# mrvollger/rustybam

Measured on AMD Instinct MI355X. Metric: CIGAR-ops/s, liftover over 100 kb sliding windows (whole pass, inputs resident in HBM), higher is better.
Workload: dtype u32

## Files before the change

### rustybam_amd/csrc/capi.hip

```cpp
#include <hip/hip_runtime.h>
#include <sys/mman.h>

#include <algorithm>
#include <cstdarg>
#include <cstdio>
#include <cstdlib>
#include <cstring>
#include <ctime>
#include <numeric>
#include <string>
#include <thread>
#include <vector>
#include <chrono>
#include <map>
#include <mutex>

#include "../../include/rustybam_amd.h"
#include "rb_lift.h"
#include "rb_trim.h"
#include "rb_launch.h"

#ifndef RB_SCAN_ROWS_MEAN_MAX
#define RB_SCAN_ROWS_MEAN_MAX 1536
#endif
#ifndef RB_SHORT_MAX_DEFAULT
#define RB_SHORT_MAX_DEFAULT 2048
#endif

#define RB_MAX_ARENA 256

#define RB_TIMING_RING 256
__global__ __launch_bounds__(256) void rb_k_fill_bytes(uint8_t *dst, uint32_t v4, size_t n) {
    const uintptr_t a = (uintptr_t)dst;
    const size_t head = n < 16 ? n : (size_t)((16 - (a & 15)) & 15);
    const size_t body = (n - head) / 16;
    const size_t tail0 = head + body * 16;
    const size_t i = (size_t)blockIdx.x * blockDim.x + threadIdx.x, stride = (size_t)gridDim.x * blockDim.x;
    for (size_t k = i; k < body; k += stride) *reinterpret_cast<uint4 *>(dst + head + k * 16) = make_uint4(v4, v4, v4, v4);
    if (i < head) dst[i] = (uint8_t)v4;
    if (i < n - tail0) dst[tail0 + i] = (uint8_t)v4;
}
extern "C" hipError_t rb_fill_async(void *dst, int value, size_t bytes, hipStream_t stream) {
    if (!bytes) return hipSuccess;
    const uint32_t b = (uint32_t)value & 255u, v4 = b | (b << 8) | (b << 16) | (b << 24);
    const size_t groups = bytes / 16 + 1;
    const unsigned blocks = (unsigned)std::min<size_t>((groups + 255) / 256, 65536);
    hipLaunchKernelGGL(rb_k_fill_bytes, dim3(blocks ? blocks : 1), dim3(256), 0, stream, (uint8_t *)dst, v4, bytes);
    return hipGetLastError();
}

struct rb_ctx {
    int device = -1;
    hipStream_t stream = nullptr;
    bool own_stream = false;
    std::string err;
    bool timing = false;
    std::vector<hipEvent_t> ev_a, ev_b;
    uint64_t timed_calls = 0;
    void *trim_scratch = nullptr;
    uint32_t trim_scratch_blocks = 0;
    void *trim_pend = nullptr;
    uint64_t trim_pend_cap = 0;
    void *scan_list = nullptr;
    uint64_t scan_list_cap = 0;
    uint64_t scan_rows_n = 0;
    void *pin[2] = {nullptr, nullptr};
    hipEvent_t pin_ev[2] = {nullptr, nullptr};
    bool pin_busy[2] = {false, false};
    unsigned pin_next = 0;
    uint64_t alloc_fallbacks = 0;
// ... 639 lines not shown
    if (!rc) rc = upload_vec(ctx, g_orig, &pl->w_orig);
    if (!rc) rc = upload_vec(ctx, o_st, &pl->wo_st);
    if (!rc) rc = upload_vec(ctx, o_en, &pl->wo_en);
    if (!rc) rc = upload_vec(ctx, cw_off, &pl->cw_off);
    if (!rc) rc = upload_vec(ctx, mono, &pl->cw_mono);
    if (!rc && pl->n_tiles) rc = upload_vec(ctx, tiles, &pl->tiles);
    if (!rc && hipStreamSynchronize(ctx->stream) != hipSuccess) rc = fail(ctx, RB_E_HIP, "plan upload: %s", hipGetErrorString(hipGetLastError()));
    if (rc) {
        rb_plan_destroy(pl);
        return rc;
    }
    *out = pl;
    return RB_OK;
}
extern "C" void rb_plan_destroy(rb_plan *pl) {
    if (!pl) return;
    void *ptrs[] = {pl->sched, pl->slot_of, pl->ident, pl->canon_pos, pl->w_st, pl->w_en, pl->w_orig, pl->wo_st, pl->wo_en, pl->cw_off, pl->cw_mono, pl->tiles};
    for (void *q : ptrs)
        if (q) (void)rb_dev_free(pl->ctx, q);
    delete pl;
}

struct ws_layout {
    size_t hit_off, win_lo, block_sums, arena, pend_count, pend_list, jobs, gen_list, x_st, x_en, bp_tmp, bp_off, bp_cur, brk_rows, copy_count, copy_list, decl_count, decl_list, gen_cp, diag_stamps, fb_count, fb_list, starts_bad, total;
};
static bool rb_no_gen_cp() {
    static const bool v = getenv("RB_DEBUG_NO_GEN_CP") != nullptr;
    return v;
}
static ws_layout ws_of(uint64_t n_rec, uint64_t rows_cap, uint64_t n_ops) {
    ws_layout w;
    size_t o = 0;
    auto take = [&](size_t bytes) {
        size_t at = o;
        o += (bytes + 255) & ~(size_t)255;
        return at;
    };
    w.hit_off = take((n_rec + 2) * 8);
    w.win_lo = take((n_rec + 2) * 4);
    w.block_sums = take(rb_scan_block_sums_count(n_rec) * 8);
    w.arena = take((size_t)RB_MAX_ARENA * RB_ARENA_STRIDE * 8);
    w.pend_count = take(256);
    w.pend_list = take((n_rec + 1) * 4);
    w.jobs = take((n_rec + 1) * sizeof(rb_job));
    w.gen_list = take((rows_cap + 1) * 4);
    w.x_st = take((rows_cap + 1) * 8);
    w.x_en = take((rows_cap + 1) * 8);
    w.bp_tmp = take((rows_cap + 1) * 8);
    w.bp_off = take((n_rec + 1) * 8);
    w.bp_cur = take((size_t)RB_MAX_ARENA * 128);
    w.brk_rows = take((rows_cap + 1) * sizeof(rb_hit_row));
    w.copy_count = take(256);
    w.copy_list = take((rows_cap + 1) * 16);
    w.decl_count = take(256);
    w.decl_list = take((n_rec + 1) * 4);
    w.gen_cp = take(rb_no_gen_cp() ? 256 : (size_t)(n_ops / RB_GCP + n_rec + 2) * sizeof(uint4));
    w.diag_stamps = take((n_rec + 1) * 4);
    w.fb_count = take(256);
    w.fb_list = take((n_rec + 1) * 4);
    w.starts_bad = take(256);
    w.total = o;
    return w;
}
extern "C" size_t rb_plan_workspace_bytes(const rb_plan *plan, uint64_t rows_cap) {
    if (!plan) return 0;
    return ws_of(plan->n_rec, rows_cap, plan->n_ops).total;
}
extern "C" size_t rb_plan_diag_stamps_offset(const rb_plan *plan, uint64_t rows_cap) {
    if (!plan) return 0;
    return ws_of(plan->n_rec, rows_cap, plan->n_ops).diag_stamps;
}

static uint64_t slot_stride_of(uint64_t n_ops, uint64_t n_rec) { return ((n_ops + 31) & ~(uint64_t)31) + 32 * n_rec + 64; }
extern "C" uint64_t rb_plan_out_capacity(const rb_plan *plan, int for_break) {
    if (!plan) return 0;
    const uint64_t slots = for_break ? std::min<uint32_t>(2u, RB_MS) : std::min<uint32_t>(plan->depth, RB_MS);
    return slots * slot_stride_of(plan->n_ops, plan->n_rec) + plan->n_ops / 16 + 32 * plan->n_rec + (1u << 20);
}

static uint32_t pick_arenas(uint64_t n_rec) {
    uint64_t a = n_rec / 256;
// ... 62 lines not shown
    p.op_starts = (policy & RB_LIFT_OP_STARTS) ? 1 : 0;
    if (p.op_starts && p.fused) return fail(ctx, RB_E_INVALID, "RB_LIFT_OP_STARTS takes finished norm_rows: not together with RB_LIFT_FUSED_SCAN");
    if (p.op_starts && (policy & RB_LIFT_DESCRIPTORS)) return fail(ctx, RB_E_INVALID, "RB_LIFT_OP_STARTS with RB_LIFT_DESCRIPTORS: a descriptor indexes the record's ORIGINAL cigar, which a batch cut in place no longer is");
    if (p.op_starts && b->n_ops > plan->n_ops) return fail(ctx, RB_E_INVALID, "RB_LIFT_OP_STARTS: batch->n_ops exceeds the plan's op count (gather the batch first)");
    if (p.op_starts && b->n_rec) {
        unsigned long long *bad = (unsigned long long *)(ws + w.starts_bad), first_bad = 0;
        HIPCHK(ctx, rb_fill_async(bad, 0xFF, 8, ctx->stream));
        HIPCHK(ctx, rb_launch_starts_check(b->op_off, norm, b->n_rec, b->n_ops, bad, ctx->stream));
        HIPCHK(ctx, hipMemcpyAsync(&first_bad, bad, 8, hipMemcpyDeviceToHost, ctx->stream));
        HIPCHK(ctx, hipStreamSynchronize(ctx->stream));
        if (first_bad != ~0ull)
            return fail(ctx, RB_E_INVALID, "RB_LIFT_OP_STARTS: record %llu lies outside the batch's %llu ops (a pass moved it: gather the batch first)",
                        first_bad, (unsigned long long)b->n_ops);
    }
    p.norm_w = const_cast<rb_norm_row *>(norm);
    p.pend_list = (uint32_t *)(ws + w.pend_list);
    p.pend_count = (unsigned long long *)(ws + w.pend_count);
    const bool use_tiles = plan->n_tiles != 0 && ((policy >> 8) & 0xFFF) == 0;
    p.tile_first = use_tiles ? plan->tiles : nullptr;
    p.n_tiles = use_tiles ? plan->n_tiles : 0;
    p.fb_list = (uint32_t *)(ws + w.fb_list);
    p.fb_count = (unsigned long long *)(ws + w.fb_count);
    const uint32_t stream_end = use_tiles ? plan->stream_end : (uint32_t)b->n_rec;
    rb_scan_params sp;
    memset(&sp, 0, sizeof sp);
    if (p.fused) {
        sp.n_rec = b->n_rec;
        sp.ops = b->ops;
        sp.op_off = b->op_off;
        sp.t_st = b->t_st, sp.t_en = b->t_en, sp.q_st = b->q_st, sp.q_en = b->q_en;
        sp.strand = b->strand;
        sp.norm_rows = p.norm_w;
        HIPCHK(ctx, rb_fill_async(p.pend_count, 0, 8, ctx->stream));
        HIPCHK(ctx, rb_launch_peek_norm(&sp, ctx->stream));
    }
    p.counters = counters;
    p.policy = policy & 1;
    p.early_exit = (policy & RB_LIFT_EARLY_EXIT) ? 1 : 0;
    p.debug_skip = (policy >> 8) & 0xFFF;
    uint64_t *block_sums = (uint64_t *)(ws + w.block_sums);
    HIPCHK(ctx, rb_fill_async(counters, 0, sizeof(rb_counters), ctx->stream));
    HIPCHK(ctx, rb_fill_async(p.copy_count, 0, 8, ctx->stream));
    HIPCHK(ctx, rb_fill_async(p.arena_cur, 0, (size_t)RB_MAX_ARENA * RB_ARENA_STRIDE * 8, ctx->stream));
    if (b->n_rec == 0) return RB_OK;
    const bool one_walk = is_break && (policy & RB_BREAK_ONE_WALK) && !p.desc_mode;
    if (one_walk) {
        p.brk_mode = 1, p.brk_max = max_size;
        p.rows_final = rows;
        p.rows = (rb_hit_row *)(ws + w.brk_rows);
        p.brk_off = (uint64_t *)(ws + w.bp_off);
        p.brk_cursor = (unsigned long long *)(ws + w.bp_cur);
        p.brk_n_arena = pick_arenas(b->n_rec);
        p.brk_arena_cap = rows_cap / p.brk_n_arena;
        p.brk_decl_list = (uint32_t *)(ws + w.decl_list);
        p.brk_decl_count = (unsigned long long *)(ws + w.decl_count);
        HIPCHK(ctx, rb_fill_async(p.brk_decl_count, 0, 8, ctx->stream));
        HIPCHK(ctx, rb_fill_async(p.brk_cursor, 0, (size_t)RB_MAX_ARENA * 128, ctx->stream));
        HIPCHK(ctx, rb_fill_async(p.hit_off, 0, (size_t)(b->n_rec + 2) * 8, ctx->stream));
        HIPCHK(ctx, rb_fill_async(p.brk_off, 0xFF, (size_t)(b->n_rec + 1) * 8, ctx->stream));
        HIPCHK(ctx, rb_launch_make_jobs(&p, ctx->stream));
        const size_t slot1 = (size_t)(ctx->timed_calls % RB_TIMING_RING);
        if (ctx->timing) HIPCHK(ctx, hipEventRecord(ctx->ev_a[slot1], ctx->stream));
        p.wave0 = 0;
        p.wave_end = stream_end;
        HIPCHK(ctx, rb_launch_liftover_stream(&p, ctx->stream));
        if (use_tiles) {
            HIPCHK(ctx, rb_fill_async(p.fb_count, 0, 8, ctx->stream));
            HIPCHK(ctx, rb_launch_liftover_tiles(&p, ctx->stream));
            HIPCHK(ctx, rb_launch_liftover_stream_list(&p, ctx->stream));
        }
        if (p.fused) {
            sp.list = p.pend_list;
            sp.n_list = (const uint64_t *)p.pend_count;
            HIPCHK(ctx, rb_launch_scan_records(&sp, ctx->stream));
        }
        if (ctx->timing) {
            HIPCHK(ctx, hipEventRecord(ctx->ev_b[slot1], ctx->stream));
            ctx->timed_calls++;
        }
        rb_break_params bp;
        memset(&bp, 0, sizeof bp);
        bp.n_rec = b->n_rec, bp.ops = b->ops, bp.op_off = b->op_off, bp.norm = norm, bp.sched = plan->sched, bp.hit_off = p.hit_off;
        bp.x_st = (uint64_t *)(ws + w.x_st), bp.x_en = (uint64_t *)(ws + w.x_en);
        bp.rows_cap = rows_cap, bp.max_size = max_size;
        bp.list = p.brk_decl_list, bp.n_list = p.brk_decl_count;
        bp.fill = 0;
        HIPCHK(ctx, rb_launch_break_list_declined(&p, ctx->stream));
        HIPCHK(ctx, rb_launch_break_pieces(&bp, ctx->stream));
        HIPCHK(ctx, rb_launch_count_and_scan(&p, block_sums, false, ctx->stream));
        bp.fill = 1;
        HIPCHK(ctx, rb_launch_break_pieces(&bp, ctx->stream));
        HIPCHK(ctx, rb_launch_break_gather(&p, ctx->stream));
        rb_lift_params pg = p;
        pg.rows = rows, pg.x_st = bp.x_st, pg.x_en = bp.x_en;
        HIPCHK(ctx, rb_launch_break_declined(&pg, ctx->stream));
        return RB_OK;
    }
    if (is_break) {
        rb_break_params bp;
        memset(&bp, 0, sizeof bp);
        bp.n_rec = b->n_rec;
        bp.ops = b->ops;
        bp.op_off = b->op_off;
        bp.norm = norm;
        bp.sched = plan->sched;
        bp.hit_off = p.hit_off;
        bp.x_st = (uint64_t *)(ws + w.x_st);
        bp.x_en = (uint64_t *)(ws + w.x_en);
        bp.rows_cap = rows_cap;
        bp.max_size = max_size;
        bp.tmp = (uint2 *)(ws + w.bp_tmp);
        bp.tmp_off = (uint64_t *)(ws + w.bp_off);
        bp.tmp_cursor = (unsigned long long *)(ws + w.bp_cur);
        bp.n_arena = pick_arenas(b->n_rec);
        bp.arena_cap = rows_cap / bp.n_arena;
        HIPCHK(ctx, rb_fill_async(bp.tmp_cursor, 0, (size_t)RB_MAX_ARENA * 128, ctx->stream));
        bp.fill = 2, bp.redo_only = 0;
        HIPCHK(ctx, rb_launch_break_pieces(&bp, ctx->stream));
        HIPCHK(ctx, rb_launch_count_and_scan(&p, block_sums, false, ctx->stream));
        HIPCHK(ctx, rb_launch_break_place(&bp, ctx->stream));
        bp.fill = 1, bp.redo_only = 1;
        HIPCHK(ctx, rb_launch_break_pieces(&bp, ctx->stream));
        p.x_st = bp.x_st;
        p.x_en = bp.x_en;
    } else {
        HIPCHK(ctx, rb_launch_count_and_scan(&p, block_sums, true, ctx->stream));
    }
    HIPCHK(ctx, rb_launch_make_jobs(&p, ctx->stream));
    const size_t slot = (size_t)(ctx->timed_calls % RB_TIMING_RING);
    if (ctx->timing) HIPCHK(ctx, hipEventRecord(ctx->ev_a[slot], ctx->stream));
    p.wave0 = 0;
    p.wave_end = stream_end;
    HIPCHK(ctx, rb_launch_liftover_stream(&p, ctx->stream));
    if (use_tiles) {
        HIPCHK(ctx, rb_fill_async(p.fb_count, 0, 8, ctx->stream));
        HIPCHK(ctx, rb_launch_liftover_tiles(&p, ctx->stream));
        HIPCHK(ctx, rb_launch_liftover_stream_list(&p, ctx->stream));
    }
    if (p.fused) {
        sp.list = p.pend_list;
        sp.n_list = (const uint64_t *)p.pend_count;
        HIPCHK(ctx, rb_launch_scan_records(&sp, ctx->stream));
    }
    if (ctx->timing) {
        HIPCHK(ctx, hipEventRecord(ctx->ev_b[slot], ctx->stream));
        ctx->timed_calls++;
    }
    HIPCHK(ctx, rb_launch_liftover_tail(&p, ctx->stream));
    return RB_OK;
}

extern "C" int rb_dev_liftover(rb_ctx *ctx, const rb_plan *plan, const rb_batch_view *batch, const rb_norm_row *norm_rows,
                               int bsearch_policy, void *workspace, rb_hit_row *rows, uint64_t rows_cap, uint32_t *out_ops,
                               uint64_t out_cap, rb_counters *counters) {
    return lift_common(ctx, plan, batch, norm_rows, bsearch_policy, workspace, rows, rows_cap, out_ops, out_cap, counters, false, 0);
}
extern "C" int rb_dev_break(rb_ctx *ctx, const rb_plan *plan, const rb_batch_view *batch, const rb_norm_row *norm_rows,
                            uint32_t max_size, int bsearch_policy, void *workspace, rb_hit_row *rows, uint64_t rows_cap,
// ... 1117 lines not shown
```

### rustybam_amd/csrc/k_liftover.hip

```cpp
#include "rb_lift.h"
#include "rb_launch.h"
#include <type_traits>
#include <algorithm>

__global__ __launch_bounds__(256) void rb_k_count_hits(rb_lift_params p) {
    const uint64_t r = (uint64_t)blockIdx.x * blockDim.x + threadIdx.x;
    if (r >= p.n_rec) return;
    uint64_t cnt = 0;
    const rb_norm_row *nr = &p.norm[r];
    const uint32_t c = p.contig[r];
    if (nr->status == RB_ST_OK && c < p.n_contig) {
        const uint64_t ws = p.cw_off[c], we = p.cw_off[c + 1];
        const uint64_t t_st = nr->t_st, t_en = nr->t_en;
        if (p.cw_mono[c]) {
            const uint64_t lo = rb_lower_en_gt(p.w_en, ws, we, t_st);
            const uint64_t hi = rb_lower_st_ge(p.w_st, ws, we, t_en);
            cnt = hi > lo ? hi - lo : 0;
            p.win_lo[r] = (uint32_t)lo;
        } else {
            for (uint64_t i = ws; i < we; i++) cnt += (t_en > p.w_st[i] && t_st < p.w_en[i]) ? 1 : 0;
        }
    }
    p.hit_off[p.canon_pos[r]] = cnt;
}

#define RB_SCAN_PER_BLOCK 2048
__global__ __launch_bounds__(256) void rb_k_scan_partial(const uint64_t *v, uint64_t n, uint64_t *block_sums) {
    __shared__ uint64_t sh[4];
    const uint64_t base = (uint64_t)blockIdx.x * RB_SCAN_PER_BLOCK;
    uint64_t s = 0;
    for (int k = 0; k < RB_SCAN_PER_BLOCK / 256; k++) {
        uint64_t i = base + (uint64_t)k * 256 + threadIdx.x;
        if (i < n) s += v[i];
    }
    s = rb_wave_sum_u64(s);
    if ((threadIdx.x & 63) == 0) sh[threadIdx.x >> 6] = s;
    __syncthreads();
    if (threadIdx.x == 0) block_sums[blockIdx.x] = sh[0] + sh[1] + sh[2] + sh[3];
}
__global__ __launch_bounds__(256) void rb_k_scan_top(uint64_t *block_sums, uint64_t n_blocks) {
    __shared__ uint64_t sh[256];
    __shared__ uint64_t carry;
    if (threadIdx.x == 0) carry = 0;
    __syncthreads();
    for (uint64_t b = 0; b < n_blocks; b += 256) {
        uint64_t i = b + threadIdx.x;
        uint64_t x = i < n_blocks ? block_sums[i] : 0;
// ... 56 lines not shown
    j.n = nr->n_ops;
    j.rec0 = p.op_off[r] + nr->first_op;
    j.t_st = nr->t_st, j.t_en = nr->t_en, j.q_st = nr->q_st, j.q_en = nr->q_en;
    const uint64_t k = p.canon_pos[r];
    const bool brk = p.brk_mode != 0;
    const uint64_t h0 = brk ? 0ull : p.hit_off[k], nh = brk ? 1ull : p.hit_off[k + 1] - h0;
    const bool explicit_w = brk || p.x_st != nullptr;
    const uint32_t cg = p.contig[r];
    const bool mono = explicit_w || (cg < p.n_contig && p.cw_mono[cg] != 0);
    uint32_t f = 0;
    const bool provisional = (nr->flags & RB_F_PROVISIONAL) != 0;
    if (nr->status == RB_ST_OK && (nh != 0 || provisional)) {
        if (h0 + nh > p.rows_cap) f |= RB_JOB_ROWS_OVERFLOW;
        else f |= RB_JOB_VALID;
    }
    if ((nr->flags & RB_F_REGULAR) || (provisional && !(nr->flags & RB_F_ENDS_NOT_MATCH))) f |= RB_JOB_REGULAR;
    if (p.strand[r] == (uint8_t)'-') f |= RB_JOB_MINUS;
    if (mono) f |= RB_JOB_MONO;
    j.flags = f;
    j.h0 = (uint32_t)h0;
    j.nh = (uint32_t)nh;
    j.lo = (explicit_w || !mono || !(f & RB_JOB_VALID) || nh == 0) ? 0u : p.win_lo[r];
    p.jobs[w] = j;
}

#define RB_RING_BASE 88
#define RB_RING_TOP_N 103
#define RB_SPILL_ROOM 4
#define RB_WPE 4, 5
#include "rb_stream.h"
#define RB_STREAM_KERNEL(NAME, BRK, DIAG, ROOM)                                                                                   \
    __global__ __launch_bounds__(256) __attribute__((amdgpu_waves_per_eu(RB_WPE), amdgpu_num_vgpr(RB_RING_BASE - (ROOM)))) void NAME(rb_lift_params p_) { \
        (void)p_;                                 \
        rb_stream_record<BRK, DIAG>();                                                                                            \
    }
RB_STREAM_KERNEL(rb_k_liftover_stream, false, false, RB_SPILL_ROOM)
RB_STREAM_KERNEL(rb_k_liftover_stream_diag, false, true, 5)

__global__ __launch_bounds__(256) void rb_k_copy_clips(rb_lift_params p) {
    const uint64_t n_copy = *p.copy_count;
    const int lane = rb_lane();
    for (uint64_t e = (uint64_t)blockIdx.x * 4u + (threadIdx.x >> 6); e < n_copy; e += (uint64_t)gridDim.x * 4u) {
        const uint4 d = p.copy_list[e];
        rb_hit_row *row = &p.rows[d.x];
        const uint32_t rec = row->rec, n = row->out_n;
        const uint32_t *src = p.ops + p.op_off[rec] + p.norm[rec].first_op + d.y;
// ... 823 lines not shown
        const uint32_t r = p.brk_decl_list[i];
        const uint64_t h0 = p.hit_off[r], n = p.hit_off[r + 1] - h0;
        for (uint64_t j = 0; j < n; j++) {
            const uint64_t h = h0 + j;
            if (h >= p.rows_cap) break;
            rb_hit_row *row = &p.rows[h];
            row->rec = r;
            row->win = (uint32_t)j;
            row->flags = RB_HIT_GENERIC;
            const unsigned long long g = atomicAdd((unsigned long long *)&p.counters->n_generic, 1ull);
            p.gen_list[g] = (uint32_t)h;
        }
    }
}
extern "C" hipError_t rb_launch_break_declined(const rb_lift_params *p, hipStream_t stream) {
    if (p->n_rec == 0) return hipSuccess;
    hipLaunchKernelGGL(rb_k_break_declined_rows, dim3((unsigned)std::min<uint64_t>((p->n_rec + 255) / 256, 256)), dim3(256), 0, stream, *p);
    if (p->gen_cp) hipLaunchKernelGGL(rb_k_generic_checkpoints, dim3(2048), dim3(256), 0, stream, *p);
    hipLaunchKernelGGL(rb_k_generic_jobs, dim3(1024), dim3(256), 0, stream, *p);
    hipLaunchKernelGGL(rb_k_liftover_generic_wave, dim3(2048), dim3(256), 0, stream, *p);
    hipLaunchKernelGGL(rb_k_finish, dim3(1), dim3(64), 0, stream, *p);
    return hipGetLastError();
}
extern "C" hipError_t rb_launch_count_and_scan(const rb_lift_params *p, uint64_t *block_sums, bool do_count, hipStream_t stream) {
    if (p->n_rec == 0) return hipSuccess;
    if (do_count) {
        const unsigned blocks = (unsigned)((p->n_rec + 255) / 256);
        hipLaunchKernelGGL(rb_k_count_hits, dim3(blocks), dim3(256), 0, stream, *p);
    }
    return rb_launch_exclusive_scan(p->hit_off, p->n_rec, block_sums, &p->counters->n_hits, stream);
}
extern "C" hipError_t rb_launch_exclusive_scan(uint64_t *v, uint64_t n, uint64_t *block_sums, uint64_t *total_out, hipStream_t stream) {
    if (n == 0) return hipSuccess;
    const uint64_t nb = (n + RB_SCAN_PER_BLOCK - 1) / RB_SCAN_PER_BLOCK;
    hipLaunchKernelGGL(rb_k_scan_partial, dim3((unsigned)nb), dim3(256), 0, stream, (const uint64_t *)v, n, block_sums);
    hipLaunchKernelGGL(rb_k_scan_top, dim3(1), dim3(256), 0, stream, block_sums, nb);
    hipLaunchKernelGGL(rb_k_scan_apply, dim3((unsigned)nb), dim3(256), 0, stream, v, n, (const uint64_t *)block_sums, total_out);
    return hipGetLastError();
}
extern "C" hipError_t rb_launch_make_jobs(const rb_lift_params *p, hipStream_t stream) {
    if (p->n_rec == 0) return hipSuccess;
    hipLaunchKernelGGL(rb_k_make_jobs, dim3((unsigned)((p->n_rec + 255) / 256)), dim3(256), 0, stream, *p);
    return hipGetLastError();
}

extern "C" hipError_t rb_launch_liftover_stream(const rb_lift_params *p, hipStream_t stream) {
    if (p->n_rec == 0 || p->wave_end <= p->wave0) return hipSuccess;
    const unsigned blocks = (unsigned)(((uint64_t)(p->wave_end - p->wave0) + 3) / 4);
    if (p->debug_skip) {
        if (!p->brk_mode) {
            hipLaunchKernelGGL(rb_k_liftover_stream_diag, dim3(blocks), dim3(256), 0, stream, *p);
            return hipGetLastError();
        }
    }
    if (p->brk_mode) return rb_launch_liftover_stream_brk(p, blocks, stream);
    hipLaunchKernelGGL(rb_k_liftover_stream, dim3(blocks), dim3(256), 0, stream, *p);
    return hipGetLastError();
}
extern "C" hipError_t rb_launch_liftover_tail(const rb_lift_params *p, hipStream_t stream) {
    if (p->n_rec == 0) return hipSuccess;
// ... 10 lines not shown
```

### rustybam_amd/csrc/k_records.hip

```cpp
#include "rb_device.h"
#include "rb_launch.h"
#include <algorithm>
#include <type_traits>

struct rb_strip {
    uint32_t lead, trail;
    uint64_t dR, dQ;
    uint64_t t_st, t_en, q_st, q_en;
};
__device__ __forceinline__ rb_strip rb_strip_ends(const uint32_t *ops, uint64_t n, uint64_t t_st, uint64_t t_en, uint64_t q_st, uint64_t q_en,
                                                  bool minus) {
    rb_strip o;
    uint64_t lead = 0, rm_st_t = 0, rm_st_q = 0;
    uint32_t prev = RB_NULL_OP;
    o.dR = o.dQ = 0;
    while (lead < n) {
        uint32_t opc, len;
        const uint32_t words = rb_op_fwd(ops, n, lead, &opc, &len);
        if (!rb_in(RB_INDEL_MASK, opc)) break;
        if (opc == RB_OP_D) {
            rm_st_t += len;
            rm_st_q += 1;
            o.dR += len;
        } else {
// ... 43 lines not shown
    w.flags = RB_F_PROVISIONAL;
    uint32_t st = RB_ST_OK;
    if (n == 0) {
        st = RB_ST_PANIC_EMPTY_CIGAR;
    } else {
        const bool minus = p.strand && p.strand[r] == (uint8_t)'-';
        const rb_strip sp = rb_strip_ends(p.ops + o0, n, p.t_st[r], p.t_en[r], p.q_st[r], p.q_en[r], minus);
        w.lead_ops = sp.lead;
        w.trail_ops = sp.trail;
        if (sp.lead || sp.trail) w.flags |= RB_F_STRIPPED;
        if ((uint64_t)sp.lead + sp.trail > n) {
            st = RB_ST_PANIC_ALL_INDEL;
        } else {
            w.t_st = sp.t_st, w.t_en = sp.t_en, w.q_st = sp.q_st, w.q_en = sp.q_en;
            w.first_op = sp.lead;
            w.n_ops = (uint32_t)(n - sp.lead - sp.trail);
            const uint32_t fo = rb_opc(p.ops[o0 + sp.lead]), lo_ = rb_opc(p.ops[o0 + n - 1 - sp.trail]);
            if (fo > 8u || lo_ > 8u || !rb_in(RB_MATCH_MASK, fo) || !rb_in(RB_MATCH_MASK, lo_)) w.flags |= RB_F_ENDS_NOT_MATCH;
        }
    }
    if (st != RB_ST_OK) w.flags &= ~(uint32_t)RB_F_PROVISIONAL;
    w.status = st;
    p.norm_rows[r] = w;
}

__device__ __forceinline__ void rb_scan_finish(const rb_scan_params &p, const uint64_t r, const uint64_t (&L)[9], const uint32_t ins_events,
                                               const uint32_t del_events, const uint32_t bad, const uint64_t o0, const uint64_t o1, const uint64_t t_st,
                                               const uint64_t t_en, const uint64_t q_st, const uint64_t q_en, const bool minus) {
    const uint64_t n = o1 - o0;
    const uint64_t R = L[RB_OP_M] + L[RB_OP_D] + L[RB_OP_N] + L[RB_OP_EQ] + L[RB_OP_X];
    const uint64_t Q = L[RB_OP_M] + L[RB_OP_I] + L[RB_OP_S] + L[RB_OP_EQ] + L[RB_OP_X];
    const uint64_t M = L[RB_OP_M] + L[RB_OP_EQ] + L[RB_OP_X];
    uint64_t U = 0;
#pragma unroll
    for (int t = 0; t < 9; t++) U += L[t];
    uint32_t flags = 0;
    if (bad == 0 && U <= 0xFFFFFFFFull) flags |= RB_F_REGULAR;
    if (L[RB_OP_M] != 0) flags |= RB_F_HAS_M;

    if (p.reduce_rows) {
        rb_reduce_row w;
        w.t_bases = R;
        w.q_bases = Q;
        w.nmatch = (uint32_t)M;
        w.aln_len = (uint32_t)U;
        w.equal = (uint32_t)L[RB_OP_EQ];
// ... 256 lines not shown
    uint64_t L[9];
    auto sum40 = [&](unsigned long long v) -> uint64_t {
        const uint32_t s_lo = rb_row_sum((uint32_t)v & 0xFFFFFu), s_hi = rb_row_sum((uint32_t)(v >> 20) & 0xFFFFFu);
        return (uint64_t)s_lo + ((uint64_t)s_hi << 20);
    };
#pragma unroll
    for (int t = 0; t < 9; t++)
        if (t != RB_OP_H && t != RB_OP_P) L[t] = sum40(hist[t][lane]);
    {
        const unsigned long long h = hist[RB_OP_H][lane], q = hist[RB_OP_P][lane];
        const uint32_t s_lo = rb_row_sum(((uint32_t)h & 0xFFFFFu) + ((uint32_t)q & 0xFFFFFu));
        const uint32_t s_hi = rb_row_sum(((uint32_t)(h >> 20) & 0xFFFFFu) + ((uint32_t)(q >> 20) & 0xFFFFFu));
        L[RB_OP_H] = (uint64_t)s_lo + ((uint64_t)s_hi << 20);
        L[RB_OP_P] = 0;
    }
    const uint32_t ins_events = rb_row_sum((uint32_t)(hist[RB_OP_I][lane] >> RB_LEN_BITS));
    const uint32_t del_events = rb_row_sum((uint32_t)(hist[RB_OP_D][lane] >> RB_LEN_BITS));
    uint32_t bad = (v_reg != 0xFFFFFFFFu ? 1u : 0u) | (v_minlen == 0u ? 2u : 0u) | (v_adj == 0u ? 4u : 0u) | v_big;
    bad = (rb_row_ballot((bad & 1u) != 0u, gbase) ? 1u : 0u) | (rb_row_ballot((bad & 2u) != 0u, gbase) ? 2u : 0u) |
          (rb_row_ballot((bad & 4u) != 0u, gbase) ? 4u : 0u) | (rb_row_ballot((bad & 8u) != 0u, gbase) ? 8u : 0u);
    if (take && gl == 0u) rb_scan_finish(p, r, L, ins_events, del_events, bad, o0, o1, t_st, t_en, q_st, q_en, minus);
}

extern "C" hipError_t rb_launch_peek_norm(const rb_scan_params *p, hipStream_t stream) {
    if (p->n_rec == 0) return hipSuccess;
    hipLaunchKernelGGL(rb_k_peek_norm, dim3((unsigned)((p->n_rec + 255) / 256)), dim3(256), 0, stream, *p);
    return hipGetLastError();
}
extern "C" hipError_t rb_launch_scan_records(const rb_scan_params *p, hipStream_t stream) {
    if (p->n_rec == 0) return hipSuccess;
    const uint64_t blocks = p->list ? std::min<uint64_t>((p->n_rec + 3) / 4, 1024) : (p->n_rec + 3) / 4;
    hipLaunchKernelGGL(rb_k_scan_records, dim3((unsigned)blocks), dim3(256), 0, stream, *p);
    return hipGetLastError();
}
extern "C" hipError_t rb_launch_scan_rows(const rb_scan_params *p, void *long_buf, hipStream_t stream) {
    if (p->n_rec == 0) return hipSuccess;
    unsigned long long *n_long = (unsigned long long *)long_buf;
    uint32_t *long_list = (uint32_t *)((char *)long_buf + 256);
    hipLaunchKernelGGL(rb_k_scan_rows, dim3((unsigned)((p->n_rec + 15) / 16)), dim3(256), 0, stream, *p, n_long, long_list);
    rb_scan_params q = *p;
    q.list = long_list, q.n_list = (const uint64_t *)n_long;
    const uint64_t blocks = std::min<uint64_t>((p->n_rec + 3) / 4, 8192);
    hipLaunchKernelGGL(rb_k_scan_records, dim3((unsigned)blocks), dim3(256), 0, stream, q);
    return hipGetLastError();
}
```

### rustybam_amd/csrc/rb_launch.h

```cpp
#pragma once
#include <hip/hip_runtime.h>
#include <stdint.h>

#include "../../include/rustybam_amd.h"

struct rb_lift_params;
struct rb_trim_params;
struct nf_read;
struct nf_tdesc;

struct rb_scan_params {
    uint64_t n_rec;
    const uint32_t *ops;
    const uint64_t *op_off;
    const uint64_t *t_st, *t_en, *q_st, *q_en;
    const uint8_t *strand;
    rb_reduce_row *reduce_rows;
    rb_norm_row *norm_rows;
    const uint32_t *list;
    const uint64_t *n_list;
};
extern "C" hipError_t rb_launch_scan_records(const rb_scan_params *p, hipStream_t stream);
extern "C" hipError_t rb_launch_scan_rows(const rb_scan_params *p, void *long_buf, hipStream_t stream);
extern "C" hipError_t rb_launch_peek_norm(const rb_scan_params *p, hipStream_t stream);

extern "C" hipError_t rb_launch_count_and_scan(const rb_lift_params *p, uint64_t *block_sums, bool do_count, hipStream_t stream);
extern "C" hipError_t rb_launch_exclusive_scan(uint64_t *v, uint64_t n, uint64_t *block_sums, uint64_t *total_out, hipStream_t stream);
extern "C" size_t rb_scan_block_sums_count(uint64_t n_rec);
extern "C" hipError_t rb_launch_make_jobs(const rb_lift_params *p, hipStream_t stream);
extern "C" hipError_t rb_launch_liftover_stream(const rb_lift_params *p, hipStream_t stream);
extern "C" hipError_t rb_launch_liftover_tail(const rb_lift_params *p, hipStream_t stream);
extern "C" hipError_t rb_launch_liftover_stream_list(const rb_lift_params *p, hipStream_t stream);
extern "C" hipError_t rb_launch_liftover_stream_brk(const rb_lift_params *p, unsigned blocks, hipStream_t stream);
extern "C" hipError_t rb_launch_liftover_tiles(const rb_lift_params *p, hipStream_t stream);
extern "C" uint32_t rb_tile_max_ops(void);
extern "C" uint32_t rb_tile_max_records(void);
extern "C" hipError_t rb_launch_break_gather(const rb_lift_params *p, hipStream_t stream);
extern "C" hipError_t rb_launch_break_declined(const rb_lift_params *p, hipStream_t stream);
extern "C" hipError_t rb_launch_break_list_declined(const rb_lift_params *p, hipStream_t stream);

struct rb_break_params {
    uint64_t n_rec;
    const uint32_t *ops;
    const uint64_t *op_off;
    const rb_norm_row *norm;
    const uint32_t *sched;
    uint64_t *hit_off;
    uint64_t *x_st, *x_en;
    uint64_t rows_cap;
    uint32_t max_size;
    int fill;
    int redo_only;
// ... 160 lines not shown
```

### rustybam_amd/csrc/rb_lift.h

```cpp
#pragma once
#include "rb_device.h"
#include <cstdlib>


#define RB_HMAX 32
#define RB_LDS_PER_HIT 6
#define RB_ARENA_STRIDE 16
#define RB_MS 2

struct __attribute__((aligned(64))) rb_job {
    uint64_t rec0;
    uint32_t n;
    uint32_t r;
    uint32_t h0;
    uint32_t flags;
    uint32_t nh;
    uint32_t lo;
    uint64_t t_st, t_en, q_st, q_en;
};
enum { RB_JOB_VALID = 1, RB_JOB_REGULAR = 2, RB_JOB_MINUS = 4, RB_JOB_MONO = 8, RB_JOB_ROWS_OVERFLOW = 16 };

struct rb_lift_params {
    uint64_t n_rec;
    const uint32_t *ops;
// ... 38 lines not shown
    uint64_t needed_base;
    uint4 *copy_list;
    unsigned long long *copy_count;
    int brk_mode;
    uint32_t brk_max;
    uint32_t brk_n_arena;
    uint64_t brk_arena_cap;
    unsigned long long *brk_cursor;
    uint64_t *brk_off;
    rb_hit_row *rows_final;
    uint32_t *brk_decl_list;
    unsigned long long *brk_decl_count;
    uint4 *gen_cp;
    uint32_t *diag_stamps;
    struct rb_gja *gj_a;
    uint4 *gj_b;
    uint2 *gj_c;
    const uint32_t *tile_first;
    uint32_t n_tiles;
    uint32_t *fb_list;
    unsigned long long *fb_count;
    int op_starts;
};
#define RB_GCP 64u
struct __attribute__((aligned(64))) rb_gja {
    uint64_t ops_off;
    uint64_t t_st, t_en, q_st, q_en;
    uint64_t wst, wen;
    uint32_t n;
    uint32_t k2;
};

typedef const __attribute__((address_space(4))) rb_lift_params *rb_kparams;
__device__ __forceinline__ rb_kparams rb_kp_here(rb_kparams q) {
    asm volatile("" : "+s"(q));
    return q;
}

__device__ __forceinline__ uint64_t rb_lower_en_gt(const uint64_t *w_en, uint64_t lo, uint64_t hi, uint64_t t_st) {
    while (lo < hi) {
        uint64_t mid = lo + ((hi - lo) >> 1);
        if (w_en[mid] > t_st) hi = mid; else lo = mid + 1;
    }
    return lo;
}
__device__ __forceinline__ uint64_t rb_lower_st_ge(const uint64_t *w_st, uint64_t lo, uint64_t hi, uint64_t t_en) {
// ... 262 lines not shown
```

Baseline: 537.4 billion.

## Fuse lift prologue: merged reset, normalize+count+job build kernel, h0 patch

Several small zero-fill launches are replaced by one reset kernel that clears a contiguous workspace region (the workspace layout is reordered so the counters sit next to each other) plus the counter struct. For the non-break path, peek-normalization, hit counting and job construction are fused into one prepare kernel that does both window binary searches in one interleaved loop. After the scan, a small kernel patches each job's h0 and flags overflow. This cuts kernel launches in the prologue. The cost is duplicated normalization logic and the risk that the fused kernel drifts from the original make_jobs semantics.

Measured after the change: 536.8 billion. About the same (-0.1%).

```diff
diff --git a/rustybam_amd/csrc/capi.hip b/rustybam_amd/csrc/capi.hip
--- a/rustybam_amd/csrc/capi.hip
+++ b/rustybam_amd/csrc/capi.hip
@@ -46,6 +46,18 @@
     const size_t groups = bytes / 16 + 1;
     const unsigned blocks = (unsigned)std::min<size_t>((groups + 255) / 256, 65536);
     hipLaunchKernelGGL(rb_k_fill_bytes, dim3(blocks ? blocks : 1), dim3(256), 0, stream, (uint8_t *)dst, v4, bytes);
+    return hipGetLastError();
+}
+
+__global__ __launch_bounds__(256) void rb_lift_reset(uint4 *a, size_t n16, unsigned long long *b, size_t n8) {
+    const size_t i = (size_t)blockIdx.x * blockDim.x + threadIdx.x;
+    if (i < n16) a[i] = make_uint4(0u, 0u, 0u, 0u);
+    if (i < n8) b[i] = 0ull;
+}
+static hipError_t rb_launch_lift_reset(void *a, size_t a_bytes, rb_counters *counters, hipStream_t stream) {
+    static_assert(sizeof(rb_counters) % 8 == 0, "rb_counters is zeroed in 8-byte words");
+    const size_t n16 = a_bytes / 16, n8 = sizeof(rb_counters) / 8;
+    hipLaunchKernelGGL(rb_lift_reset, dim3((unsigned)((std::max(n16, n8) + 255) / 256)), dim3(256), 0, stream, (uint4 *)a, n16, (unsigned long long *)counters, n8);
     return hipGetLastError();
 }
 
@@ -731,6 +743,7 @@
 }
 
 struct ws_layout {
+    size_t reset_lift, reset_brk;
     size_t hit_off, win_lo, block_sums, arena, pend_count, pend_list, jobs, gen_list, x_st, x_en, bp_tmp, bp_off, bp_cur, brk_rows, copy_count, copy_list, decl_count, decl_list, gen_cp, diag_stamps, fb_count, fb_list, starts_bad, total;
 };
 static bool rb_no_gen_cp() {
@@ -748,8 +761,14 @@
     w.hit_off = take((n_rec + 2) * 8);
     w.win_lo = take((n_rec + 2) * 4);
     w.block_sums = take(rb_scan_block_sums_count(n_rec) * 8);
+    w.pend_count = take(256);
+    w.copy_count = take(256);
     w.arena = take((size_t)RB_MAX_ARENA * RB_ARENA_STRIDE * 8);
-    w.pend_count = take(256);
+    w.fb_count = take(256);
+    w.reset_lift = o - w.pend_count;
+    w.decl_count = take(256);
+    w.bp_cur = take((size_t)RB_MAX_ARENA * 128);
+    w.reset_brk = o - w.pend_count;
     w.pend_list = take((n_rec + 1) * 4);
     w.jobs = take((n_rec + 1) * sizeof(rb_job));
     w.gen_list = take((rows_cap + 1) * 4);
@@ -757,15 +776,11 @@
     w.x_en = take((rows_cap + 1) * 8);
     w.bp_tmp = take((rows_cap + 1) * 8);
     w.bp_off = take((n_rec + 1) * 8);
-    w.bp_cur = take((size_t)RB_MAX_ARENA * 128);
     w.brk_rows = take((rows_cap + 1) * sizeof(rb_hit_row));
-    w.copy_count = take(256);
     w.copy_list = take((rows_cap + 1) * 16);
-    w.decl_count = take(256);
     w.decl_list = take((n_rec + 1) * 4);
     w.gen_cp = take(rb_no_gen_cp() ? 256 : (size_t)(n_ops / RB_GCP + n_rec + 2) * sizeof(uint4));
     w.diag_stamps = take((n_rec + 1) * 4);
-    w.fb_count = take(256);
     w.fb_list = take((n_rec + 1) * 4);
     w.starts_bad = take(256);
     w.total = o;
@@ -874,6 +889,11 @@
     p.fb_list = (uint32_t *)(ws + w.fb_list);
     p.fb_count = (unsigned long long *)(ws + w.fb_count);
     const uint32_t stream_end = use_tiles ? plan->stream_end : (uint32_t)b->n_rec;
+    p.counters = counters;
+    p.policy = policy & 1;
+    p.early_exit = (policy & RB_LIFT_EARLY_EXIT) ? 1 : 0;
+    p.debug_skip = (policy >> 8) & 0xFFF;
+    HIPCHK(ctx, rb_launch_lift_reset(ws + w.pend_count, is_break ? w.reset_brk : w.reset_lift, counters, ctx->stream));
     rb_scan_params sp;
     memset(&sp, 0, sizeof sp);
     if (p.fused) {
@@ -883,17 +903,9 @@
         sp.t_st = b->t_st, sp.t_en = b->t_en, sp.q_st = b->q_st, sp.q_en = b->q_en;
         sp.strand = b->strand;
         sp.norm_rows = p.norm_w;
-        HIPCHK(ctx, rb_fill_async(p.pend_count, 0, 8, ctx->stream));
-        HIPCHK(ctx, rb_launch_peek_norm(&sp, ctx->stream));
-    }
-    p.counters = counters;
-    p.policy = policy & 1;
-    p.early_exit = (policy & RB_LIFT_EARLY_EXIT) ? 1 : 0;
-    p.debug_skip = (policy >> 8) & 0xFFF;
+        if (is_break) HIPCHK(ctx, rb_launch_peek_norm(&sp, ctx->stream));
+    }
     uint64_t *block_sums = (uint64_t *)(ws + w.block_sums);
-    HIPCHK(ctx, rb_fill_async(counters, 0, sizeof(rb_counters), ctx->stream));
-    HIPCHK(ctx, rb_fill_async(p.copy_count, 0, 8, ctx->stream));
-    HIPCHK(ctx, rb_fill_async(p.arena_cur, 0, (size_t)RB_MAX_ARENA * RB_ARENA_STRIDE * 8, ctx->stream));
     if (b->n_rec == 0) return RB_OK;
     const bool one_walk = is_break && (policy & RB_BREAK_ONE_WALK) && !p.desc_mode;
     if (one_walk) {
@@ -906,8 +918,6 @@
         p.brk_arena_cap = rows_cap / p.brk_n_arena;
         p.brk_decl_list = (uint32_t *)(ws + w.decl_list);
         p.brk_decl_count = (unsigned long long *)(ws + w.decl_count);
-        HIPCHK(ctx, rb_fill_async(p.brk_decl_count, 0, 8, ctx->stream));
-        HIPCHK(ctx, rb_fill_async(p.brk_cursor, 0, (size_t)RB_MAX_ARENA * 128, ctx->stream));
         HIPCHK(ctx, rb_fill_async(p.hit_off, 0, (size_t)(b->n_rec + 2) * 8, ctx->stream));
         HIPCHK(ctx, rb_fill_async(p.brk_off, 0xFF, (size_t)(b->n_rec + 1) * 8, ctx->stream));
         HIPCHK(ctx, rb_launch_make_jobs(&p, ctx->stream));
@@ -917,7 +927,6 @@
         p.wave_end = stream_end;
         HIPCHK(ctx, rb_launch_liftover_stream(&p, ctx->stream));
         if (use_tiles) {
-            HIPCHK(ctx, rb_fill_async(p.fb_count, 0, 8, ctx->stream));
             HIPCHK(ctx, rb_launch_liftover_tiles(&p, ctx->stream));
             HIPCHK(ctx, rb_launch_liftover_stream_list(&p, ctx->stream));
         }
@@ -939,7 +948,7 @@
         bp.fill = 0;
         HIPCHK(ctx, rb_launch_break_list_declined(&p, ctx->stream));
         HIPCHK(ctx, rb_launch_break_pieces(&bp, ctx->stream));
-        HIPCHK(ctx, rb_launch_count_and_scan(&p, block_sums, false, ctx->stream));
+        HIPCHK(ctx, rb_launch_hit_scan(&p, block_sums, ctx->stream));
         bp.fill = 1;
         HIPCHK(ctx, rb_launch_break_pieces(&bp, ctx->stream));
         HIPCHK(ctx, rb_launch_break_gather(&p, ctx->stream));
@@ -966,26 +975,29 @@
         bp.tmp_cursor = (unsigned long long *)(ws + w.bp_cur);
         bp.n_arena = pick_arenas(b->n_rec);
         bp.arena_cap = rows_cap / bp.n_arena;
-        HIPCHK(ctx, rb_fill_async(bp.tmp_cursor, 0, (size_t)RB_MAX_ARENA * 128, ctx->stream));
         bp.fill = 2, bp.redo_only = 0;
         HIPCHK(ctx, rb_launch_break_pieces(&bp, ctx->stream));
-        HIPCHK(ctx, rb_launch_count_and_scan(&p, block_sums, false, ctx->stream));
+        HIPCHK(ctx, rb_launch_hit_scan(&p, block_sums, ctx->stream));
         HIPCHK(ctx, rb_launch_break_place(&bp, ctx->stream));
         bp.fill = 1, bp.redo_only = 1;
         HIPCHK(ctx, rb_launch_break_pieces(&bp, ctx->stream));
         p.x_st = bp.x_st;
         p.x_en = bp.x_en;
+        HIPCHK(ctx, rb_launch_make_jobs(&p, ctx->stream));
     } else {
-        HIPCHK(ctx, rb_launch_count_and_scan(&p, block_sums, true, ctx->stream));
-    }
-    HIPCHK(ctx, rb_launch_make_jobs(&p, ctx->stream));
+        rb_prep_params pp;
+        pp.l = p;
+        pp.t_st = b->t_st, pp.t_en = b->t_en, pp.q_st = b->q_st, pp.q_en = b->q_en;
+        HIPCHK(ctx, rb_launch_lift_prepare(&pp, p.fused != 0, ctx->stream));
+        HIPCHK(ctx, rb_launch_hit_scan(&p, block_sums, ctx->stream));
+        HIPCHK(ctx, rb_launch_jobs_h0(&p, ctx->stream));
+    }
     const size_t slot = (size_t)(ctx->timed_calls % RB_TIMING_RING);
     if (ctx->timing) HIPCHK(ctx, hipEventRecord(ctx->ev_a[slot], ctx->stream));
     p.wave0 = 0;
     p.wave_end = stream_end;
     HIPCHK(ctx, rb_launch_liftover_stream(&p, ctx->stream));
     if (use_tiles) {
-        HIPCHK(ctx, rb_fill_async(p.fb_count, 0, 8, ctx->stream));
         HIPCHK(ctx, rb_launch_liftover_tiles(&p, ctx->stream));
         HIPCHK(ctx, rb_launch_liftover_stream_list(&p, ctx->stream));
     }
diff --git a/rustybam_amd/csrc/k_liftover.hip b/rustybam_amd/csrc/k_liftover.hip
--- a/rustybam_amd/csrc/k_liftover.hip
+++ b/rustybam_amd/csrc/k_liftover.hip
@@ -2,27 +2,6 @@
 #include "rb_launch.h"
 #include <type_traits>
 #include <algorithm>
-
-__global__ __launch_bounds__(256) void rb_k_count_hits(rb_lift_params p) {
-    const uint64_t r = (uint64_t)blockIdx.x * blockDim.x + threadIdx.x;
-    if (r >= p.n_rec) return;
-    uint64_t cnt = 0;
-    const rb_norm_row *nr = &p.norm[r];
-    const uint32_t c = p.contig[r];
-    if (nr->status == RB_ST_OK && c < p.n_contig) {
-        const uint64_t ws = p.cw_off[c], we = p.cw_off[c + 1];
-        const uint64_t t_st = nr->t_st, t_en = nr->t_en;
-        if (p.cw_mono[c]) {
-            const uint64_t lo = rb_lower_en_gt(p.w_en, ws, we, t_st);
-            const uint64_t hi = rb_lower_st_ge(p.w_st, ws, we, t_en);
-            cnt = hi > lo ? hi - lo : 0;
-            p.win_lo[r] = (uint32_t)lo;
-        } else {
-            for (uint64_t i = ws; i < we; i++) cnt += (t_en > p.w_st[i] && t_st < p.w_en[i]) ? 1 : 0;
-        }
-    }
-    p.hit_off[p.canon_pos[r]] = cnt;
-}
 
 #define RB_SCAN_PER_BLOCK 2048
 __global__ __launch_bounds__(256) void rb_k_scan_partial(const uint64_t *v, uint64_t n, uint64_t *block_sums) {
@@ -125,6 +104,19 @@
     j.nh = (uint32_t)nh;
     j.lo = (explicit_w || !mono || !(f & RB_JOB_VALID) || nh == 0) ? 0u : p.win_lo[r];
     p.jobs[w] = j;
+}
+
+__global__ __launch_bounds__(256) void rb_k_jobs_h0(rb_lift_params p) {
+    const uint64_t r = (uint64_t)blockIdx.x * blockDim.x + threadIdx.x;
+    if (r >= p.n_rec) return;
+    const uint64_t k = p.canon_pos[r];
+    rb_job *j = &p.jobs[p.slot_of[r]];
+    const uint64_t h0 = p.hit_off[k], nh = p.hit_off[k + 1] - h0;
+    j->h0 = (uint32_t)h0;
+    if (h0 + nh > p.rows_cap) {
+        const uint32_t f = j->flags;
+        if (f & RB_JOB_VALID) j->flags = (f & ~(uint32_t)RB_JOB_VALID) | RB_JOB_ROWS_OVERFLOW, j->lo = 0u;
+    }
 }
 
 #define RB_RING_BASE 88
@@ -994,12 +986,8 @@
     hipLaunchKernelGGL(rb_k_finish, dim3(1), dim3(64), 0, stream, *p);
     return hipGetLastError();
 }
-extern "C" hipError_t rb_launch_count_and_scan(const rb_lift_params *p, uint64_t *block_sums, bool do_count, hipStream_t stream) {
+extern "C" hipError_t rb_launch_hit_scan(const rb_lift_params *p, uint64_t *block_sums, hipStream_t stream) {
     if (p->n_rec == 0) return hipSuccess;
-    if (do_count) {
-        const unsigned blocks = (unsigned)((p->n_rec + 255) / 256);
-        hipLaunchKernelGGL(rb_k_count_hits, dim3(blocks), dim3(256), 0, stream, *p);
-    }
     return rb_launch_exclusive_scan(p->hit_off, p->n_rec, block_sums, &p->counters->n_hits, stream);
 }
 extern "C" hipError_t rb_launch_exclusive_scan(uint64_t *v, uint64_t n, uint64_t *block_sums, uint64_t *total_out, hipStream_t stream) {
@@ -1008,6 +996,11 @@
     hipLaunchKernelGGL(rb_k_scan_partial, dim3((unsigned)nb), dim3(256), 0, stream, (const uint64_t *)v, n, block_sums);
     hipLaunchKernelGGL(rb_k_scan_top, dim3(1), dim3(256), 0, stream, block_sums, nb);
     hipLaunchKernelGGL(rb_k_scan_apply, dim3((unsigned)nb), dim3(256), 0, stream, v, n, (const uint64_t *)block_sums, total_out);
+    return hipGetLastError();
+}
+extern "C" hipError_t rb_launch_jobs_h0(const rb_lift_params *p, hipStream_t stream) {
+    if (p->n_rec == 0) return hipSuccess;
+    hipLaunchKernelGGL(rb_k_jobs_h0, dim3((unsigned)((p->n_rec + 255) / 256)), dim3(256), 0, stream, *p);
     return hipGetLastError();
 }
 extern "C" hipError_t rb_launch_make_jobs(const rb_lift_params *p, hipStream_t stream) {
diff --git a/rustybam_amd/csrc/k_records.hip b/rustybam_amd/csrc/k_records.hip
--- a/rustybam_amd/csrc/k_records.hip
+++ b/rustybam_amd/csrc/k_records.hip
@@ -1,4 +1,5 @@
 #include "rb_device.h"
+#include "rb_lift.h"
 #include "rb_launch.h"
 #include <algorithm>
 #include <type_traits>
@@ -89,6 +90,101 @@
     if (st != RB_ST_OK) w.flags &= ~(uint32_t)RB_F_PROVISIONAL;
     w.status = st;
     p.norm_rows[r] = w;
+}
+
+template <bool PEEK>
+__global__ __launch_bounds__(256) void rb_k_lift_prepare(rb_prep_params pp) {
+    const rb_lift_params &p = pp.l;
+    const uint64_t r64 = (uint64_t)blockIdx.x * blockDim.x + threadIdx.x;
+    if (r64 >= p.n_rec) return;
+    const uint32_t r = (uint32_t)r64;
+    const uint64_t o0 = p.op_off[r];
+    const uint32_t cg = p.contig[r];
+    const bool minus = p.strand[r] == (uint8_t)'-';
+    const uint64_t k = p.canon_pos[r];
+    const uint64_t slot = p.slot_of[r];
+    const bool cok = cg < p.n_contig;
+    rb_norm_row w;
+    uint64_t ws = 0, we = 0;
+    uint32_t mono_c = 0;
+    if constexpr (PEEK) {
+        const uint64_t n = p.op_off[r + 1] - o0;
+        const uint64_t t_st = pp.t_st[r], t_en = pp.t_en[r], q_st = pp.q_st[r], q_en = pp.q_en[r];
+        uint32_t fw = RB_NULL_OP, lw = RB_NULL_OP;
+        if (n) fw = p.ops[o0], lw = p.ops[o0 + n - 1];
+        if (cok) ws = p.cw_off[cg], we = p.cw_off[cg + 1], mono_c = p.cw_mono[cg];
+        w.t_st = w.t_en = w.q_st = w.q_en = 0;
+        w.first_op = w.n_ops = w.lead_ops = w.trail_ops = w.nmatch = w.aln_len = 0;
+        w.flags = RB_F_PROVISIONAL;
+        uint32_t st = RB_ST_OK;
+        const uint32_t fo = rb_opc(fw), lo_ = rb_opc(lw);
+        if (n == 0) {
+            st = RB_ST_PANIC_EMPTY_CIGAR;
+        } else if (fo <= 8u && lo_ <= 8u && rb_in(RB_MATCH_MASK, fo) && rb_in(RB_MATCH_MASK, lo_)) {
+            w.t_st = t_st, w.t_en = t_en, w.q_st = q_st, w.q_en = q_en;
+            w.n_ops = (uint32_t)n;
+        } else {
+            const rb_strip sp = rb_strip_ends(p.ops + o0, n, t_st, t_en, q_st, q_en, minus);
+            w.lead_ops = sp.lead;
+            w.trail_ops = sp.trail;
+            if (sp.lead || sp.trail) w.flags |= RB_F_STRIPPED;
+            if ((uint64_t)sp.lead + sp.trail > n) {
+                st = RB_ST_PANIC_ALL_INDEL;
+            } else {
+                w.t_st = sp.t_st, w.t_en = sp.t_en, w.q_st = sp.q_st, w.q_en = sp.q_en;
+                w.first_op = sp.lead;
+                w.n_ops = (uint32_t)(n - sp.lead - sp.trail);
+                const uint32_t f2 = rb_opc(p.ops[o0 + sp.lead]), l2 = rb_opc(p.ops[o0 + n - 1 - sp.trail]);
+                if (f2 > 8u || l2 > 8u || !rb_in(RB_MATCH_MASK, f2) || !rb_in(RB_MATCH_MASK, l2)) w.flags |= RB_F_ENDS_NOT_MATCH;
+            }
+        }
+        if (st != RB_ST_OK) w.flags &= ~(uint32_t)RB_F_PROVISIONAL;
+        w.status = st;
+        p.norm_w[r] = w;
+    } else {
+        w = p.norm[r];
+        if (cok) ws = p.cw_off[cg], we = p.cw_off[cg + 1], mono_c = p.cw_mono[cg];
+    }
+    uint64_t cnt = 0, lo = 0;
+    if (w.status == RB_ST_OK && cok) {
+        if (mono_c) {
+            uint64_t lo1 = ws, hi1 = we, lo2 = ws, hi2 = we;
+            while (lo1 < hi1 || lo2 < hi2) {
+                const bool a1 = lo1 < hi1, a2 = lo2 < hi2;
+                const uint64_t m1 = lo1 + ((hi1 - lo1) >> 1), m2 = lo2 + ((hi2 - lo2) >> 1);
+                const uint64_t v1 = a1 ? p.w_en[m1] : 0, v2 = a2 ? p.w_st[m2] : 0;
+                if (a1) {
+                    if (v1 > w.t_st) hi1 = m1; else lo1 = m1 + 1;
+                }
+                if (a2) {
+                    if (v2 >= w.t_en) hi2 = m2; else lo2 = m2 + 1;
+                }
+            }
+            lo = lo1;
+            cnt = lo2 > lo1 ? lo2 - lo1 : 0;
+            p.win_lo[r] = (uint32_t)lo;
+        } else {
+            for (uint64_t i = ws; i < we; i++) cnt += (w.t_en > p.w_st[i] && w.t_st < p.w_en[i]) ? 1 : 0;
+        }
+    }
+    p.hit_off[k] = cnt;
+    rb_job j;
+    j.r = r;
+    j.n = w.n_ops;
+    j.rec0 = o0 + w.first_op;
+    j.t_st = w.t_st, j.t_en = w.t_en, j.q_st = w.q_st, j.q_en = w.q_en;
+    const bool mono = cok && mono_c != 0;
+    const bool provisional = (w.flags & RB_F_PROVISIONAL) != 0;
+    uint32_t f = 0;
+    if (w.status == RB_ST_OK && (cnt != 0 || provisional)) f |= RB_JOB_VALID;
+    if ((w.flags & RB_F_REGULAR) || (provisional && !(w.flags & RB_F_ENDS_NOT_MATCH))) f |= RB_JOB_REGULAR;
+    if (minus) f |= RB_JOB_MINUS;
+    if (mono) f |= RB_JOB_MONO;
+    j.flags = f;
+    j.h0 = 0;
+    j.nh = (uint32_t)cnt;
+    j.lo = (!mono || !(f & RB_JOB_VALID) || cnt == 0) ? 0u : (uint32_t)lo;
+    p.jobs[slot] = j;
 }
 
 __device__ __forceinline__ void rb_scan_finish(const rb_scan_params &p, const uint64_t r, const uint64_t (&L)[9], const uint32_t ins_events,
@@ -391,6 +487,13 @@
     if (take && gl == 0u) rb_scan_finish(p, r, L, ins_events, del_events, bad, o0, o1, t_st, t_en, q_st, q_en, minus);
 }
 
+extern "C" hipError_t rb_launch_lift_prepare(const rb_prep_params *p, bool peek, hipStream_t stream) {
+    if (p->l.n_rec == 0) return hipSuccess;
+    const dim3 grid((unsigned)((p->l.n_rec + 255) / 256));
+    if (peek) hipLaunchKernelGGL(rb_k_lift_prepare<true>, grid, dim3(256), 0, stream, *p);
+    else hipLaunchKernelGGL(rb_k_lift_prepare<false>, grid, dim3(256), 0, stream, *p);
+    return hipGetLastError();
+}
 extern "C" hipError_t rb_launch_peek_norm(const rb_scan_params *p, hipStream_t stream) {
     if (p->n_rec == 0) return hipSuccess;
     hipLaunchKernelGGL(rb_k_peek_norm, dim3((unsigned)((p->n_rec + 255) / 256)), dim3(256), 0, stream, *p);
diff --git a/rustybam_amd/csrc/rb_launch.h b/rustybam_amd/csrc/rb_launch.h
--- a/rustybam_amd/csrc/rb_launch.h
+++ b/rustybam_amd/csrc/rb_launch.h
@@ -5,6 +5,7 @@
 #include "../../include/rustybam_amd.h"
 
 struct rb_lift_params;
+struct rb_prep_params;
 struct rb_trim_params;
 struct nf_read;
 struct nf_tdesc;
@@ -23,11 +24,13 @@
 extern "C" hipError_t rb_launch_scan_records(const rb_scan_params *p, hipStream_t stream);
 extern "C" hipError_t rb_launch_scan_rows(const rb_scan_params *p, void *long_buf, hipStream_t stream);
 extern "C" hipError_t rb_launch_peek_norm(const rb_scan_params *p, hipStream_t stream);
-
-extern "C" hipError_t rb_launch_count_and_scan(const rb_lift_params *p, uint64_t *block_sums, bool do_count, hipStream_t stream);
+extern "C" hipError_t rb_launch_lift_prepare(const rb_prep_params *p, bool peek, hipStream_t stream);
+
+extern "C" hipError_t rb_launch_hit_scan(const rb_lift_params *p, uint64_t *block_sums, hipStream_t stream);
 extern "C" hipError_t rb_launch_exclusive_scan(uint64_t *v, uint64_t n, uint64_t *block_sums, uint64_t *total_out, hipStream_t stream);
 extern "C" size_t rb_scan_block_sums_count(uint64_t n_rec);
 extern "C" hipError_t rb_launch_make_jobs(const rb_lift_params *p, hipStream_t stream);
+extern "C" hipError_t rb_launch_jobs_h0(const rb_lift_params *p, hipStream_t stream);
 extern "C" hipError_t rb_launch_liftover_stream(const rb_lift_params *p, hipStream_t stream);
 extern "C" hipError_t rb_launch_liftover_tail(const rb_lift_params *p, hipStream_t stream);
 extern "C" hipError_t rb_launch_liftover_stream_list(const rb_lift_params *p, hipStream_t stream);
diff --git a/rustybam_amd/csrc/rb_lift.h b/rustybam_amd/csrc/rb_lift.h
--- a/rustybam_amd/csrc/rb_lift.h
+++ b/rustybam_amd/csrc/rb_lift.h
@@ -84,6 +84,10 @@
     unsigned long long *fb_count;
     int op_starts;
 };
+struct rb_prep_params {
+    rb_lift_params l;
+    const uint64_t *t_st, *t_en, *q_st, *q_en;
+};
 #define RB_GCP 64u
 struct __attribute__((aligned(64))) rb_gja {
     uint64_t ops_off;
```
